# lucidrains/dreamer4

Hardware: AMD Instinct MI355X
Metric: imagined latent steps/sec (higher is better)
Workload: dtype f32; 1 GPU; cfg2 Moving-MNIST-latent shape: dim=512 depth=6 heads=8x64 latents=32x32 spatial=4 registers=8; generate(H+1=16 frames, num_steps=4, time cache) + learn_from_experience(ppo) + clip/AdamW both heads; global_batch=256, per_gpu_batch=256, horizon=15, num_steps=4, parallelism=dp1

## Files before the change

### dreamer4_amd/_lib.py

```python
from __future__ import annotations

import ctypes as C
import os

_HERE = os.path.dirname(os.path.abspath(__file__))
LIB_PATH = os.path.join(_HERE, 'libd4hip.so')

D4_MAX_ACTION_TYPES = 8

GEMM_RMS_ROWSCALE, GEMM_SILU, GEMM_SWIGLU, GEMM_TRANS_A, GEMM_TRANS_B, GEMM_ACCUMULATE = 1, 2, 4, 8, 16, 32


class Config(C.Structure):
    _fields_ = [
        ('dim', C.c_int32), ('dim_latent', C.c_int32), ('num_latent_tokens', C.c_int32), ('depth', C.c_int32),
        ('time_block_every', C.c_int32), ('attn_heads', C.c_int32), ('attn_dim_head', C.c_int32),
        ('attn_softclamp_value', C.c_float),
        ('num_spatial_tokens', C.c_int32), ('num_register_tokens', C.c_int32), ('max_steps', C.c_int32),
        ('num_tasks', C.c_int32), ('num_discrete_action_types', C.c_int32),
        ('num_discrete_actions', C.c_int32 * D4_MAX_ACTION_TYPES), ('num_continuous_actions', C.c_int32),
        ('multi_token_pred_len', C.c_int32),
        ('policy_head_mlp_depth', C.c_int32), ('value_head_mlp_depth', C.c_int32),
        ('terminal_mlp_depth', C.c_int32), ('predict_terminals', C.c_int32),
        ('reward_num_bins', C.c_int32), ('value_num_bins', C.c_int32), ('reward_encoder_type', C.c_int32), ('matmul_bf16', C.c_int32), ('head_mlp_recipe', C.c_int32), ('continuous_beta_param', C.c_int32),
# ... 168 lines not shown
    'd4_gemm_split': (_I, [_P, _I, _P, _L, _I, _P, _I, _P, _P, _I, _I, _I, _I, _I, _F, _I, _P]),
    'd4_split_f16x2': (_I, [_P, _P, _I, _I, _I, _L, _P, _P]),
    'd4_row_scale_exp': (_I, [_P, _L, _I, _I, _P, _P]),
    'd4_gemm_split2': (_I, [_P, _I, _P, _L, _I, _P, _P, _I, _P, _P, _I, _I, _I, _I, _I, _F, _I, _P, _P]),
    'd4_rmsnorm': (_I, [_P, _I, _P, _P, _I, _I, _I, _F, _P]),
    'd4_small_attn': (_I, [_P, _L, _L] * 4 + [_P] + [_P, _L, _L] * 3 + [_P] + [_I] * 4 + [_F] + [_I] * 6 + [_P]),
    'd4_small_attn_wide': (_I, [_P, _L, _L] * 4 + [_P] + [_P, _L, _L] * 3 + [_P] + [_I] * 4 + [_F] + [_I] * 6 + [_P]),
    'd4_small_attn_wide_bf16': (_I, [_P, _L, _L] * 4 + [_P] + [_P, _L, _L] * 3 + [_P] + [_I] * 4 + [_F] + [_I] * 6 + [_P]),
    'd4_pool_mix': (_I, [_P, _I, _P, _I, _P, _P, _I, _P, _I, _P, _P, _I, _I, _I, _F, _P, _P, _P, _P, _P]),
    'd4_pool_mix_deep': (_I, [_P, _I, _P, _I, _P, _P, _I, _P, _I, _P, _P, _I, _I, _I, _F, _P, _P, _P, _P, _P]),
    'd4_time_attn_decode': (_I, [_P, _I, _P, _I, _P, _P, _P, _P, _I, _P] + [_I] * 8 + [_P, _F, _I, _I, _P]),
    'd4_gemm_family_configs': (_I, [_I]),
    'd4_gemm_run': (_I, [C.POINTER(GemmDesc), _I, _I, _P]),
    'd4_gemm_run_rowmap': (_I, [C.POINTER(GemmDesc), _I, _I, _I, _I, _I, _I, _P]),
    'd4_gemm_run_pair': (_I, [C.POINTER(GemmDesc), C.POINTER(GemmDesc), _I, _I, _P]),
    'd4_gemm_fill_capacity': (_I, [C.POINTER(GemmDesc)]),
    'd4_gemm_run_fill': (_I, [C.POINTER(GemmDesc), C.POINTER(GemmDesc), _I, _P]),
    'd4_gemm_run_fill_rowmap': (_I, [C.POINTER(GemmDesc), C.POINTER(GemmDesc), _I, _I, _I, _I, _I, _P]),
    'd4_tile16_weights': (_I, [_P, _I, _P, _I, _I, _P]),
    'd4_frame_attn_out': (_I, [_P, _L, _L] * 4 + [_P] + [_P, _L, _L] * 2 + [_P] + [_I] * 3 + [_F] + [_I] * 3 + [_P, _I, _P, _I, _P, _I, _P, _I, _I, _I, _I, _P]),
    'd4_attn_out_cols': (_I, [_P, _L, _L] * 4 + [_P] + [_P, _L, _L] * 2 + [_P] + [_I] * 3 + [_F] + [_I] * 3 + [_P, _I, _I, _P, _I, _P, _I, _P, _I, _I, _I, _I, _P]),
    'd4_frame_pool': (_I, [_P, _I, _P, _I, _P, _P, _I, _P, _I, _P, _I, _I, _I, _F, _P, _P, _I, _I, _P, _I, _P, _I, _P, _I, _I, _I, _I, _P]),
    'd4_frame_pool_tail': (_I, [_P, _P, _P, _I, _I, _I, _I, _P, _I, _P, _I, _P, _I, _I, _I, _I, _P]),
    'd4_lqap_in': (_I, [_P, _I, _P, _I, _P, _P, _P, _P] + [_I] * 5 + [_F, _P]),
    'd4_lqap_out': (_I, [_P, _I, _P, _P, _P, _P, _I, _P, _I] + [_I] * 5 + [_P]),
    'd4_debug_last_form': (C.c_char_p, [C.c_char_p]),
    'd4_debug_forms': (_I, [C.c_char_p, _I, C.POINTER(C.c_char_p)]),
    'd4_train_attn_core_plane_floats': (C.c_size_t, [_I] * 3),
    'd4_train_xattn_core_plane_floats': (C.c_size_t, [_I] * 4),
    'd4_train_attn_core': (_I, [_P, _I] + [_P] * 7 + [_I] * 4 + [_F, _I, _I, _I, _L, _L, _I, _P, _I, _P, C.c_size_t, _P]),
# ... 90 lines not shown
```

### dreamer4_amd/csrc/abi_ops.hip

```cpp
#include "common.h"
#include "engine.h"
#include "prof.h"

extern "C" {

int d4_profile_bf16_enable(int stride) { d4::gemm_bf16_profile_enable(stride); return 0; }
int d4_profile_bf16_read(double* ms, double* flops, int64_t* count) { return d4::gemm_bf16_profile_read(ms, flops, count); }
int d4_profile_enable(int on) { return d4::gemm_profile_enable(on); }
int d4_profile_read(double* ms, double* flops, int64_t* count, int nclass) { return d4::gemm_profile_read(ms, flops, count, nclass); }
int d4_profile_classes(void) { return d4::gemm_profile_classes(); }
int d4_profile_glue_enable(int mask) { return d4::glue_profile_enable(mask); }
int d4_profile_glue_read(double* ms, double* bytes, int64_t* count, int nclass) { return d4::glue_profile_read(ms, bytes, count, nclass); }
int d4_profile_glue_classes(void) { return d4::GL_N; }
int d4_profile_glue_read_flops(double* flops, int nclass) { return d4::glue_profile_read_flops(flops, nclass); }
const char* d4_profile_glue_class_name(int c) { return d4::glue_class_name(c); }
int d4_frame_fused_set(int mode) { return d4::frame_fused_set(mode); }
const char* d4_profile_class_name(int c) { return d4::gemm_profile_class_name(c); }

int d4_gemm(const float* A, int lda, const float* W, int ldw, float* C, int ldc, const float* bias,
            const float* R, int ldr, int M, int N, int K, int flags, float rms_eps, void* stream) {
    d4::GemmArgs g{A, lda, W, ldw, C, ldc, bias, R, ldr, M, N, K, flags, rms_eps};
    return d4::gemm(g, static_cast<hipStream_t>(stream));
}

// ... 403 lines not shown
            D4_REQUIRE(al16(a) && al16(b) && d4::gemm_skinny_pair_applicable(a, b),
                       "d4_gemm_run_pair: call not supported (gemm_skinny_pair_applicable: two few-row products of equal K, no SiLU-GLU, batch or mirror weights)");
            return d4::gemm_skinny_pair(a, b, s);
        case D4_PAIR_BF16A:
            D4_REQUIRE(d4::gemm_bf16a_pair_applicable(a, b),
                       "d4_gemm_run_pair: call not supported (gemm_bf16a_pair_applicable: equal K, flags == RMS, no bias / R / C2 / batch, a 64 x 64 or 128 x 64 tile by the rule)");
            return d4::gemm_bf16a_pair_launch(a, b, s);
        case D4_PAIR_V2:
            D4_REQUIRE(al16(a) && al16(b) && !a.Wb && !b.Wb && a.K == b.K && d4::gemm2_pair_config_ok(config) && d4::gemm2_pair_applicable(a, b) &&
                       d4::gemm2_config_valid(config, a) && d4::gemm2_config_valid(config, b),
                       "d4_gemm_run_pair: call not supported (gemm2 pair configuration %d: gemm2_pair_config_ok / gemm2_pair_applicable)", config);
            return d4::gemm2_pair_launch(config, a, b, s);
    }
    D4_REQUIRE(false, "d4_gemm_run_pair: unknown target %d", target);
}

int d4_tile16_weights(const float* W, int ldw, float* Wt, int N, int K, void* stream) {
    D4_REQUIRE(W && Wt && N >= 16 && K >= 4 && ldw >= K && ((uintptr_t)W % 16) == 0 && ((uintptr_t)Wt % 16) == 0, "d4_tile16_weights: bad arguments");
    return d4::tile16_weights(W, ldw, Wt, N, K, static_cast<hipStream_t>(stream));
}
static d4::SmallAttnArgs frame_attn_args(const float* q, int64_t q_group_stride, int64_t q_item_stride, const float* k, int64_t k_group_stride, int64_t k_item_stride,
                                         const float* v, int64_t v_group_stride, int64_t v_item_stride, const float* gate, int64_t g_group_stride, int64_t g_item_stride,
                                         const float* k_gamma, const float* vres, int64_t r_group_stride, int64_t r_item_stride, const float* mix, int64_t m_group_stride,
                                         int64_t m_item_stride, uint16_t* out_b, int frames, int heads, int S, float softclamp, int mask_special, int belief, int dh) {
    d4::SmallAttnArgs sa{};
    sa.q = q; sa.q_group_stride = q_group_stride; sa.q_item_stride = q_item_stride;
    sa.k = k; sa.k_group_stride = k_group_stride; sa.k_item_stride = k_item_stride;
    sa.v = v; sa.v_group_stride = v_group_stride; sa.v_item_stride = v_item_stride;
    sa.gate = gate; sa.g_group_stride = g_group_stride; sa.g_item_stride = g_item_stride;
    sa.k_gamma = k_gamma;
// ... 81 lines not shown
```

### dreamer4_amd/csrc/engine.hip

```cpp
#include "common.h"
#include "engine.h"
#include "prof.h"
#include <math.h>
#include <stdarg.h>
#include <stdio.h>
#include <stdlib.h>
#include <string.h>
#include <memory>

using namespace d4;

namespace d4 {

static constexpr float RMS_EPS = 1.1920928955078125e-07f;

static int round_up(int v, int m) { return (v + m - 1) / m * m; }

int engine_layout(d4_engine* e, bool assign) {
    const d4_config& c = e->c;
    size_t off = 0;
    auto alloc_bytes = [&](size_t bytes) -> char* {
        off = (off + 255) / 256 * 256;
        char* p = assign ? e->ws + off : nullptr;
        off += bytes;
// ... 725 lines not shown
    int32_t offs[D4_MAX_ACTION_TYPES] = {0}, sizes[D4_MAX_ACTION_TYPES] = {0};
    int o = 0;
    for (int a = 0; a < e->na; ++a) { offs[a] = o; sizes[a] = c.num_discrete_actions[a]; o += sizes[a]; }
    D4_HIP(hipMemcpyAsync(e->action_offsets, offs, sizeof(offs), hipMemcpyHostToDevice, s));
    D4_HIP(hipMemcpyAsync(e->action_sizes, sizes, sizeof(sizes), hipMemcpyHostToDevice, s));
    D4_HIP(hipStreamSynchronize(s));
    e->prepared = true;
    return 0;
}

static GemmArgs ff_in_call(const d4_engine* e, const FfPrep& fp, const float* x, int ldx, int rows) {
    return GemmArgs{x, ldx, fp.w1, e->D, e->ffh, e->inner_pad, fp.b1, nullptr, 0, rows, 2 * e->inner_pad, e->D,
                    GEMM_RMS_ROWSCALE | GEMM_SWIGLU, RMS_EPS, 2.0 * rows * (2.0 * e->inner) * e->D};
}

static int ff_block(const EvalCtx& cx, d4_engine* e, const FfPrep& fp, const float* out_b, const float* x, int ldx, float* y, int ldy,
                    int rows, float* y_compact = nullptr, int S = 0, int has_agent = 1, const GemmArgs* fill = nullptr) {
    int rc;
    GemmArgs g1 = ff_in_call(e, fp, x, ldx, rows);
    if (fill) {
        trunk_call(cx.img, g1);
        if ((rc = gemm_x3sk_fill(g1, *fill, gemm_x3sk_fill_tiles(*fill), cx.s))) return rc;
    } else
    if ((rc = engine_gemm(cx, g1))) return rc;
    GemmArgs g2{e->ffh, e->inner_pad, fp.w2, e->inner_pad, y, ldy, out_b, x, ldx, rows, e->D, e->inner_pad, 0, RMS_EPS,
                2.0 * rows * (double)e->D * e->inner};
    if (y_compact) { g2.C2 = y_compact; g2.ldc2 = e->D; g2.c2_S = S; g2.c2_lo = cx.keep_lo; g2.c2_hi = cx.keep_hi; g2.c2_last = has_agent; }
    return engine_gemm(cx, g2);
}

int g_pool_wide_keys = 1;
int g_rollout_clean_agent_row = 1;
int g_rollout_batched_heads = 1;
int g_lqap_in_fused = 1;
int g_lqap_out_fused = 1;
int g_last_layer_compact_q = 1;
int g_layer0_const_rows = 1;
int g_pool_const_keys = 1;
int g_ff_fill_pool_keys = 1;
unsigned g_launch_count = 0;
static GemmArgs pool_key_call(d4_engine* e, int p, const float* hiddens, int L, int M, int rule_M, float* keys0) {
    const int D = e->D, hp = e->hp;
    GemmArgs gk{hiddens, D, e->pkv_w[p], D, e->pool_kv, hp, nullptr, nullptr, 0, L * M, hp, D, GEMM_RMS_ROWSCALE, RMS_EPS};
    gk.rule_M = L * rule_M;
    if (keys0) { gk.A = hiddens + (size_t)M * D; gk.C = keys0 + (size_t)M * hp; gk.M = (L - 1) * M; gk.rule_M = L * M; }
    return gk;
}

static int pool_block(const EvalCtx& cx, d4_engine* e, int p, const float* x, float* y, int L, int M, const float* hiddens = nullptr,
                      float* y_compact = nullptr, int S = 0, int has_agent = 1, int rule_M = 0, float* keys0 = nullptr, int keys_done = 0) {
    if (!hiddens) hiddens = e->slabs;
    const d4_config& c = e->c;
    const int D = e->D, hp = e->hp;
    const AttnW& a = e->pools[p];
// ... 266 lines not shown
            GemmArgs g1 = ff_in_call(e, e->ffp[l], h1, D, M);
            trunk_call(cx.img, g1);
            const int cap = gemm_rule_takes_x3sk(g1) ? gemm_x3sk_fill_capacity(g1) : 0;
            const GemmArgs gk = pool_key_call(e, l, e->slabs, L, M, 0, keys0(l));
            const int ready = (gk.M - M) / 128;
            const int per_block = (e->hp + 63) / 64;
            const int blocks = cap / per_block < ready ? cap / per_block : ready;
            if (blocks > 0 && takes(v2, L * M, e->hp, D, GEMM_RMS_ROWSCALE, e->pkv_w[l]) &&
                takes(v2, gk.M - 128 * blocks, e->hp, D, GEMM_RMS_ROWSCALE, e->pkv_w[l], L * M)) {
                keys_done = 128 * blocks;
                kfill = gk;
                kfill.M = keys_done; kfill.rule_M = 0;
                D4_REQUIRE(gemm_x3sk_fill_applicable(kfill), "ff_fill_pool_keys: the key problem of pool %d is no fill problem", l);
            }
        }
        if ((rc = ff_block(cx, e, e->ffp[l], e->layer_ff[l].out_b, h1, D, h2, D, M, cslab(2 * l + 2), S, has_agent, keys_done ? &kfill : nullptr))) return rc;
        if (l != c.depth - 1) {
            float* xc = compact_tail_at(l + 1) ? e->xpool_c : nullptr;
            if ((rc = pool_block(cx, e, l, h2, e->xpool, 2 * l + 3, M, nullptr, xc, S, has_agent, 0, keys0(l), keys_done))) return rc;
            x_in = e->xpool;
        }
    }

    float* xfc = e->xfc;
    const float* last = slab(2 * c.depth);
    if ((rc = copy_rows(cslab(2 * c.depth), D, xfc, D, Mc, D, s))) return rc;
    if (e->encoder) {
        const int P = e->P;
        const float* spec = cslab(2 * c.depth);
        if ((rc = gemm_simple(cx, spec, D, e->cq_w, D, e->cq, e->ldcq, Mc, hd + h, D, GEMM_RMS_ROWSCALE, nullptr, nullptr, 0))) return rc;
        if ((rc = gemm_simple(cx, last, D, e->ckv_w, D, e->ckv, 2 * hd, M, 2 * hd, D, GEMM_RMS_ROWSCALE, nullptr, nullptr, 0))) return rc;
        SmallAttnArgs sa{};
        sa.dh = c.attn_dim_head;
        sa.q = e->cq; sa.q_group_stride = (int64_t)n * e->ldcq; sa.q_item_stride = e->ldcq;
// ... 404 lines not shown
    D4_REQUIRE(!io->sample_actions || e->nc == 0 || (io->actions_cont && io->beta_noise && io->log_probs_cont && io->cont_params), "sample_actions needs the continuous action outputs and beta_noise");
    D4_REQUIRE(!io->sample_actions || io->values, "sample_actions needs the values output");
    D4_REQUIRE(!io->sample_terminals || (c.predict_terminals && io->bern_u), "sample_terminals needs predict_terminals and bern_u");
    D4_REQUIRE(io->use_time_cache || io->noise_context || T - P <= 1, "noise_context is required without the time cache");
    const int F = T - P;
    const int step_size = c.max_steps / K;
    int sl, rc;
    if ((rc = step_log2_of(step_size, &sl))) return rc;
    if ((rc = check_step_log2(e, sl))) return rc;
    const int n_el = c.num_latent_tokens * c.dim_latent;
    const int D = e->D, S = e->S, A = e->A, na = e->na, nc = e->nc;
    if (!io->use_time_cache) e->cache_frames = 0;
    const bool lean = d4::g_rollout_clean_agent_row != 0;
    const int lean_keep = (lean && d4::engine_clean_agent_only(e)) ? 1 : c.num_spatial_tokens + 1;
    const int variant = (lean ? 1 : 0) | (d4::g_lqap_in_fused ? 2 : 0) | (d4::g_lqap_out_fused ? 4 : 0) | (d4::g_last_layer_compact_q ? 8 : 0) |
                        (d4::g_layer0_const_rows ? 16 : 0) | (d4::g_pool_const_keys ? 32 : 0) | (d4::g_ff_fill_pool_keys ? 64 : 0);
    const float* hist = nullptr;
    if (d4::g_rollout_batched_heads && F >= 1 && F <= e->head_rows) {
        if (io->agent_embed) hist = io->agent_embed;
        else if (F == 1) hist = e->agent_c;
        else if ((size_t)B * F <= e->hist_rows) hist = e->agent_hist;
    }
    const bool heads_after = hist != nullptr;

    for (int f = 0; f < F; ++f) {
        const int cur = P + f;
        int Tq, t0;
        bool commit;
        if (io->use_time_cache && (e->cache_frames > 0 || cur == 0)) { Tq = 1; t0 = e->cache_frames; commit = true; }
        else if (io->use_time_cache) { Tq = cur + 1; t0 = 0; commit = true; }
        else { Tq = cur + 1; t0 = 0; commit = false; }
// ... 122 lines not shown
}


int d4_debug_switch(const char* name, int value) {
    int* sw = nullptr;
    if (name && !strcmp(name, "launch_count")) {
        const int old = (int)(d4::g_launch_count & 0x7fffffffu);
        d4::g_launch_count = (unsigned)value;
        return old;
    }
    if (name && !strcmp(name, "ff_fill_launches")) {
        const int old = (int)(d4::g_fill_launches & 0x7fffffffu);
        d4::g_fill_launches = (unsigned)value;
        return old;
    }
    if (name && !strcmp(name, "time_attn_fused_append")) sw = &d4::g_time_attn_fused_append;
    else if (name && !strcmp(name, "rollout_clean_agent_row")) sw = &d4::g_rollout_clean_agent_row;
    else if (name && !strcmp(name, "rollout_batched_heads")) sw = &d4::g_rollout_batched_heads;
    else if (name && !strcmp(name, "attn_out_cols")) sw = &d4::g_attn_out_cols;
    else if (name && !strcmp(name, "lqap_in_fused")) sw = &d4::g_lqap_in_fused;
    else if (name && !strcmp(name, "lqap_out_fused")) sw = &d4::g_lqap_out_fused;
    else if (name && !strcmp(name, "last_layer_compact_q")) sw = &d4::g_last_layer_compact_q;
    else if (name && !strcmp(name, "layer0_const_rows")) sw = &d4::g_layer0_const_rows;
    else if (name && !strcmp(name, "pool_const_keys")) sw = &d4::g_pool_const_keys;
    else if (name && !strcmp(name, "ff_fill_pool_keys")) sw = &d4::g_ff_fill_pool_keys;
    else if (name && !strcmp(name, "pool_wide_keys")) sw = &d4::g_pool_wide_keys;
    else if (name && !strcmp(name, "pool_mix_deep")) sw = &d4::g_pool_mix_deep;
    else if (name && !strcmp(name, "time_attn_tiled")) sw = &d4::g_time_attn_tiled;
    else if (name && !strcmp(name, "space_attn_tiled")) sw = &d4::g_space_attn_tiled;
    else if (name && !strcmp(name, "cross_attn_tiled")) sw = &d4::g_cross_attn_tiled;
    else if (name && !strcmp(name, "small_attn_wide")) sw = &d4::g_small_attn_wide;
    if (!sw) return -1;
    const int old = *sw;
    *sw = value;
    return old;
}
int d4_gemm_force_config(int id) {
    d4::gemm_bf16a_force_config(-1);
    d4::gemm_bf16_force_config(-1);
    const int n_main = d4::gemm_force_config(-1);
// ... 33 lines not shown
```

### dreamer4_amd/csrc/gemm.hip

```cpp
#include "common.h"
#include <string.h>
#include <hip/hip_ext.h>
#include "kernels.h"
#include <mutex>
#include <math.h>
#include <stdio.h>
#include <stdlib.h>
#include <map>
#include <tuple>
#include <type_traits>
#include <vector>

namespace d4 {


template <int BM, int BN, int WGM, int WGN, int BK, int KS, bool TA, bool TB, bool KTAIL>
__global__ __launch_bounds__(WGM * WGN * 64 * KS) void gemm_kernel(GemmArgs p) {
    constexpr int LDS_LD = BK + 4;
    constexpr int RF4 = BK / 4;
    constexpr int NT = WGM * WGN * 64 * KS;
    constexpr int TM = BM / WGM / 32;
    constexpr int TN = BN / WGN / 32;
    static_assert(TM >= 1 && TN >= 1, "tile");
    constexpr int A_F4 = BM * BK / 4 / NT;
// ... 797 lines not shown
    D4_TUNE_STRICT_CHECK(p, nb);
    int best = 0;
    if (int rc = autotune_v4(p, stream, &best)) return rc;
    g_tuned4[key] = best;
    tune_cache_append(key, 400 + best);
    return launch_v4(best, p, stream);
}

bool gemm_h2_takes(const GemmArgs& p) {
    if (!p.Wb || p.wplane <= 0 || !p.wscale || !gemm_h2_applicable(p) || gemm_skinny_applicable(p)) return false;
    if (g_forced_cfg >= 0 && g_forced_cfg < 400) return false;
    if (g_forced_cfg >= 400) return true;
    return p.M >= 256 && p.K >= 128 && p.N >= 64 && (double)p.M * p.N * p.K * (p.batch > 0 ? p.batch : 1) >= 1.2e9;
}

int gemm_pair(const GemmArgs& a_in, const GemmArgs& b_in, hipStream_t stream) {
    std::lock_guard<std::recursive_mutex> lock(gemm_mutex());
    GemmArgs a = a_in, b = b_in;
    if (int rc = gemm_rowmap_refused(a, "gemm_pair")) return rc;
    if (int rc = gemm_rowmap_refused(b, "gemm_pair")) return rc;
    const bool fp32_rule = (!a.Wb || (a.wplane > 0 && a.N < 2048)) && (!b.Wb || (b.wplane > 0 && b.N < 2048)) &&
                           !gemm_h2_takes(a) && !gemm_h2_takes(b);
    if (fp32_rule && g_forced_cfg < 0 && a.M > 0 && b.M > 0 && a.K == b.K && use_v2(a) && use_v2(b) && !gemm_skinny_applicable(a) &&
        !gemm_skinny_applicable(b) && gemm2_pair_applicable(a, b)) {
        a.Wb = nullptr; a.wplane = 0; a.wscale = nullptr; b.Wb = nullptr; b.wplane = 0; b.wscale = nullptr;
        const GemmArgs& big = (double)a.M * a.N >= (double)b.M * b.N ? a : b;
        tune_cache_load();
        auto it = g_tuned2.find(TuneKey{big.M, big.N, big.K, big.flags, big.batch});
        const int c = it != g_tuned2.end() ? it->second : heuristic_v2(big);
        if (gemm2_pair_config_ok(c) && gemm2_config_valid(c, a) && gemm2_config_valid(c, b)) {
            const int cls = N_TILE_CFG + c;
            const bool timed = ((g_prof_mask >> cls) & 1) && (g_prof_tick++ % g_prof_stride) == 0;
            if (!timed) return gemm2_pair_launch(c, a, b, stream);
            ProfRec rec{};
            rec.a = prof_event(); rec.b = prof_event(); rec.cls = cls;
// ... 97 lines not shown
```

### dreamer4_amd/csrc/gemm2.hip

```cpp
#include "common.h"
#include <hip/hip_ext.h>
#include "kernels.h"
#include "gemm2_body.h"
#include <stdlib.h>
#include <type_traits>

namespace d4 {

template <int WGM, int WGN, int TM, int TN, int NS, int BK, bool RMS>
__global__ __launch_bounds__(WGM* WGN * 64) void gemm2_kernel(GemmArgs p) {
    gemm2_body<WGM, WGN, TM, TN, NS, BK, RMS>(p, blockIdx.x, blockIdx.y);
}

template <int WGM, int WGN, int TM, int TN, int NS, int BK, bool RMS>
__global__ __launch_bounds__(WGM* WGN * 64) void gemm2_rowmap_kernel(GemmArgs p) {
    gemm2_body<WGM, WGN, TM, TN, NS, BK, RMS, true>(p, blockIdx.x, blockIdx.y);
}

template <int WGM, int WGN, int TM, int TN, int NS, int BK, bool RMS>
__global__ __launch_bounds__(WGM* WGN * 64) void gemm2_pair_kernel(GemmArgs a, GemmArgs b, int nblk_a) {
    const int bid = blockIdx.x;
    if (bid < nblk_a) gemm2_body<WGM, WGN, TM, TN, NS, BK, RMS>(a, bid, 0);
    else gemm2_body<WGM, WGN, TM, TN, NS, BK, RMS>(b, bid - nblk_a, 0);
}

constexpr int KS_GROUPS = 4, KS_NS = 3, KS_BM = 32, KS_BN = 64, KS_BK = 32;
constexpr int KS_STAGE_F = (KS_BM + KS_BN) * KS_BK;
constexpr int KS_RING_F = KS_NS * KS_STAGE_F;
constexpr int KS_LDP = KS_BN + 4;

__global__ __launch_bounds__(1024) void gemm2_ksplit_kernel(GemmArgs p) {
    constexpr int BK = KS_BK, CH = 8, RPP = 8, BM = KS_BM, BN = KS_BN, NS = KS_NS, LPW = 3, NSLOT = (BM + BN) / RPP;
    extern __shared__ __attribute__((aligned(16))) float smem[];
    const int tid = threadIdx.x, lane = tid & 63;
    const int wave = __builtin_amdgcn_readfirstlane(tid >> 6);
    const int grp = wave >> 2, w = wave & 3, wm = w >> 1, wn = w & 1;
    int bid = blockIdx.x;
    const int nbn = (p.N + BN - 1) / BN, nbm = (p.M + BM - 1) / BM;
// ... 206 lines not shown
int gemm2_pair_launch(int c, const GemmArgs& a, const GemmArgs& b, hipStream_t stream, hipEvent_t ea, hipEvent_t eb) {
    if (int rc = gemm_rowmap_refused(a, "gemm2 pair")) return rc;
    if (int rc = gemm_rowmap_refused(b, "gemm2 pair")) return rc;
    D4_REQUIRE(gemm2_pair_applicable(a, b) && gemm2_config_valid(c, a) && gemm2_config_valid(c, b), "gemm2 pair: configuration %d is not valid for these calls", c);
    switch (c) {
        case V2_64x64: return launch2_pair<2, 2, 2, 2, 3, 32>(a, b, stream, ea, eb);
        case V2_128x64_8: return launch2_pair<4, 2, 2, 2, 3, 32>(a, b, stream, ea, eb);
        case V2_128x64_k16: return launch2_pair<4, 2, 2, 2, 4, 16>(a, b, stream, ea, eb);
        case V2_32x64: return launch2_pair<2, 2, 1, 2, 3, 32>(a, b, stream, ea, eb);
        case V2_32x32: return launch2_pair<2, 2, 1, 1, 3, 32>(a, b, stream, ea, eb);
        case V2_64x32: return launch2_pair<4, 1, 1, 2, 3, 32>(a, b, stream, ea, eb);
    }
    return 2;
}

int gemm2_launch(int c, const GemmArgs& p, hipStream_t stream, hipEvent_t ea, hipEvent_t eb) {
    D4_REQUIRE(gemm2_config_valid(c, p), "gemm2: configuration %d is not valid for this call", c);
    switch (c) {
        case V2_64x64: return launch2<2, 2, 2, 2, 3, 32>(p, stream, ea, eb);
        case V2_64x64_s: return launch2<4, 1, 1, 4, 3, 32>(p, stream, ea, eb);
        case V2_128x64_8: return launch2<4, 2, 2, 2, 3, 32>(p, stream, ea, eb);
        case V2_128x64_s: return launch2<4, 1, 2, 4, 3, 32>(p, stream, ea, eb);
        case V2_128x64_k16: return launch2<4, 2, 2, 2, 4, 16>(p, stream, ea, eb);
        case V2_128x128_k16: return launch2<4, 2, 2, 4, 3, 16>(p, stream, ea, eb);
        case V2_32x64: return launch2<2, 2, 1, 2, 3, 32>(p, stream, ea, eb);
        case V2_32x64_s: return launch2<2, 1, 1, 4, 3, 32>(p, stream, ea, eb);
        case V2_32x32: return launch2<2, 2, 1, 1, 3, 32>(p, stream, ea, eb);
        case V2_64x32: return launch2<4, 1, 1, 2, 3, 32>(p, stream, ea, eb);
    }
    return 2;
// ... 4 lines not shown
```

### dreamer4_amd/csrc/kernels.h

```cpp
#pragma once
#include <hip/hip_runtime.h>
#include <stdint.h>

namespace d4 {

enum : int {
    GEMM_RMS_ROWSCALE = 1,
    GEMM_SILU = 2,
    GEMM_SWIGLU = 4,
    GEMM_TRANS_A = 8,
    GEMM_TRANS_B = 16,
    GEMM_ACCUMULATE = 32,
};

struct GemmArgs {
    const float* A; int lda;
    const float* W; int ldw;
    float* C; int ldc;
    const float* bias;
    const float* R; int ldr;
    int M, N, K;
    int flags;
    float rms_eps;
    double algo_flops = 0;
// ... 67 lines not shown
int gemm_x3sk_fill_launch(const GemmArgs& main, const GemmArgs& fill, int fill_tiles, hipStream_t stream, hipEvent_t ea = nullptr, hipEvent_t eb = nullptr);
extern unsigned g_fill_launches;
int gemm_x3sk_fill(const GemmArgs& main, const GemmArgs& fill, int fill_tiles, hipStream_t stream);
bool gemm2_applicable(const GemmArgs& p);
bool gemm2_config_valid(int c, const GemmArgs& p);
int gemm2_configs();
const char* gemm2_config_name(int c);
void gemm2_config_tile(int c, int* bm, int* bn);
int gemm2_launch(int c, const GemmArgs& p, hipStream_t stream, hipEvent_t ea = nullptr, hipEvent_t eb = nullptr);
bool gemm2_ksplit_applicable(const GemmArgs& p);
bool gemm2_ksplit_rule(const GemmArgs& p);
int gemm2_ksplit_launch(const GemmArgs& p, hipStream_t stream, hipEvent_t ea = nullptr, hipEvent_t eb = nullptr);
bool gemm2_pair_config_ok(int c);
bool gemm2_pair_applicable(const GemmArgs& a, const GemmArgs& b);
int gemm2_pair_launch(int c, const GemmArgs& a, const GemmArgs& b, hipStream_t stream, hipEvent_t ea = nullptr, hipEvent_t eb = nullptr);
int gemm_pair(const GemmArgs& a, const GemmArgs& b, hipStream_t stream);
bool gemm_skinny_applicable(const GemmArgs& p);
int gemm_skinny(const GemmArgs& p, hipStream_t stream);
bool gemm_skinny_pair_applicable(const GemmArgs& a, const GemmArgs& b);
int gemm_skinny_pair(const GemmArgs& a, const GemmArgs& b, hipStream_t stream);
int gemm_profile_enable(int on);
bool gemm_profile_active();
int gemm_profile_read(double* ms, double* flops, int64_t* count, int nclass);
int gemm_profile_classes();
extern int g_time_attn_fused_append;
extern int g_pool_wide_keys;
extern int g_attn_out_cols;
extern int g_time_attn_tiled;
extern int g_space_attn_tiled;
extern int g_cross_attn_tiled;
extern int g_small_attn_wide;
// ... 211 lines not shown
```

### include/d4hip.h

```cpp
#ifndef D4HIP_H
#define D4HIP_H

#include <stddef.h>
#include <stdint.h>

#ifdef __cplusplus
extern "C" {
#endif

#define D4_MAX_ACTION_TYPES 8
#define D4_MODE_DYNAMICS 0
#define D4_MODE_DECODER 1
#define D4_MODE_ENCODER 2
#define D4_MLP_PRE_RMS 0
#define D4_MLP_POST_LAYER 1
#define D4_BETA_SOFTPLUS_P1 0
#define D4_BETA_EXP_P1 1

typedef struct d4_config {
    int32_t dim, dim_latent, num_latent_tokens, depth, time_block_every;
    int32_t attn_heads, attn_dim_head;
    float attn_softclamp_value;
    int32_t num_spatial_tokens, num_register_tokens, max_steps, num_tasks;
    int32_t num_discrete_action_types;
// ... 309 lines not shown
#define D4_GEMM_H2 5
#define D4_GEMM_SKINNY 6
#define D4_GEMM_BF16 7
#define D4_GEMM_BF16A 8
#define D4_GEMM_FAMILIES 9
int d4_gemm_family_configs(int family);
int d4_gemm_run(const d4_gemm_desc* d, int family, int config, void* stream);
int d4_gemm_run_rowmap(const d4_gemm_desc* d, int family, int config, int rm_Sc, int rm_S, int rm_lo, int rm_nr, void* stream);
int d4_gemm_fill_capacity(const d4_gemm_desc* main_call);
int d4_gemm_run_fill(const d4_gemm_desc* main_call, const d4_gemm_desc* fill, int fill_tiles, void* stream);
int d4_gemm_run_fill_rowmap(const d4_gemm_desc* main_call, const d4_gemm_desc* fill, int fill_tiles, int rm_Sc, int rm_S, int rm_lo, int rm_nr, void* stream);
#define D4_PAIR_SKINNY 0
#define D4_PAIR_BF16A 1
#define D4_PAIR_V2 2
int d4_gemm_run_pair(const d4_gemm_desc* a, const d4_gemm_desc* b, int target, int config, void* stream);
int d4_tile16_weights(const float* W, int ldw, float* Wt, int N, int K, void* stream);
int d4_frame_attn_out(const float* q, int64_t q_group_stride, int64_t q_item_stride, const float* k, int64_t k_group_stride, int64_t k_item_stride,
                      const float* v, int64_t v_group_stride, int64_t v_item_stride, const float* gate, int64_t g_group_stride, int64_t g_item_stride,
                      const float* k_gamma, const float* vres, int64_t r_group_stride, int64_t r_item_stride, const float* mix, int64_t m_group_stride,
                      int64_t m_item_stride, uint16_t* out_b, int frames, int heads, int S, float softclamp, int mask_special, int belief, int dh,
                      const float* wo_t, int D, const float* resid, int ldr, float* out, int ldo, float* c2, int ldc2, int c2_lo, int c2_hi, int c2_last,
                      void* stream);
int d4_attn_out_cols(const float* q, int64_t q_group_stride, int64_t q_item_stride, const float* k, int64_t k_group_stride, int64_t k_item_stride,
                     const float* v, int64_t v_group_stride, int64_t v_item_stride, const float* gate, int64_t g_group_stride, int64_t g_item_stride,
                     const float* k_gamma, const float* vres, int64_t r_group_stride, int64_t r_item_stride, const float* mix, int64_t m_group_stride,
                     int64_t m_item_stride, uint16_t* out_b, int frames, int heads, int S, float softclamp, int mask_special, int belief, int dh,
                     const float* W, int ldw, int D, const float* resid, int ldr, float* out, int ldo, float* c2, int ldc2, int c2_lo, int c2_hi, int c2_last,
                     void* stream);
int d4_frame_pool(const float* q, int ldq, const float* x, int ldx, const float* gate_w, const float* k, int ldk, const float* hid, int D,
                  const float* k_gamma, int M, int L, int heads, float eps, const float* wv_t, const float* wo_t, int frames, int S, const float* resid,
// ... 135 lines not shown
```

Before: 23620 imagined steps/s.

## Pair FF output GEMM with old pool-key GEMM in one mixed-RMS launch

Adds a paired GEMM kernel where one half runs without the RMS row scale and the other with it. In the dynamics forward pass it uses this kernel to compute the pool-key projection of older rows together with the feed-forward output GEMM of each non-final layer. The aim is fewer launches and better occupancy from co-scheduling a skinny GEMM with a larger independent one. In exchange it adds another kernel variant, a switch, and extra eligibility checks on the host.

Result: no change. 23810 imagined steps/s (median of 6 runs) (+0.8%).

```diff
diff --git a/dreamer4_amd/_lib.py b/dreamer4_amd/_lib.py
--- a/dreamer4_amd/_lib.py
+++ b/dreamer4_amd/_lib.py
@@ -206,6 +206,8 @@
     'd4_gemm_run': (_I, [C.POINTER(GemmDesc), _I, _I, _P]),
     'd4_gemm_run_rowmap': (_I, [C.POINTER(GemmDesc), _I, _I, _I, _I, _I, _I, _P]),
     'd4_gemm_run_pair': (_I, [C.POINTER(GemmDesc), C.POINTER(GemmDesc), _I, _I, _P]),
+    'd4_gemm_run_pair_mixed': (_I, [C.POINTER(GemmDesc), C.POINTER(GemmDesc), _I, _P]),
+    'd4_gemm_run_pair_mixed_rowmap': (_I, [C.POINTER(GemmDesc), C.POINTER(GemmDesc), _I, _I, _I, _I, _I, _P]),
     'd4_gemm_fill_capacity': (_I, [C.POINTER(GemmDesc)]),
     'd4_gemm_run_fill': (_I, [C.POINTER(GemmDesc), C.POINTER(GemmDesc), _I, _P]),
     'd4_gemm_run_fill_rowmap': (_I, [C.POINTER(GemmDesc), C.POINTER(GemmDesc), _I, _I, _I, _I, _I, _P]),
diff --git a/dreamer4_amd/csrc/abi_ops.hip b/dreamer4_amd/csrc/abi_ops.hip
--- a/dreamer4_amd/csrc/abi_ops.hip
+++ b/dreamer4_amd/csrc/abi_ops.hip
@@ -441,6 +441,24 @@
     }
     D4_REQUIRE(false, "d4_gemm_run_pair: unknown target %d", target);
 }
+static int gemm_run_pair_mixed_args(const d4::GemmArgs& a, const d4::GemmArgs& b, int config, void* stream) {
+    auto al16 = [](const d4::GemmArgs& g) { return ((uintptr_t)g.A % 16) == 0 && ((uintptr_t)g.W % 16) == 0 && (g.lda % 4) == 0 && (g.ldw % 4) == 0; };
+    D4_REQUIRE(al16(a) && al16(b) && !a.Wb && !b.Wb, "d4_gemm_run_pair_mixed: call not supported (operands must be 16-byte aligned f32 matrices, no mirror weights)");
+    return d4::gemm2_pair_mixed_launch(config, a, b, static_cast<hipStream_t>(stream));
+}
+int d4_gemm_run_pair_mixed(const d4_gemm_desc* da, const d4_gemm_desc* db, int config, void* stream) {
+    if (int rc = gemm_desc_check("d4_gemm_run_pair_mixed", da)) return rc;
+    if (int rc = gemm_desc_check("d4_gemm_run_pair_mixed", db)) return rc;
+    return gemm_run_pair_mixed_args(gemm_args_of(*da), gemm_args_of(*db), config, stream);
+}
+int d4_gemm_run_pair_mixed_rowmap(const d4_gemm_desc* da, const d4_gemm_desc* db, int config, int rm_Sc, int rm_S, int rm_lo, int rm_nr, void* stream) {
+    if (int rc = gemm_desc_check("d4_gemm_run_pair_mixed_rowmap", da)) return rc;
+    if (int rc = gemm_desc_check("d4_gemm_run_pair_mixed_rowmap", db)) return rc;
+    D4_REQUIRE(rm_Sc >= 1 && rm_nr >= 0 && rm_lo >= 0 && rm_lo <= rm_Sc && rm_S == rm_Sc + rm_nr && rm_S <= 65535, "d4_gemm_run_pair_mixed_rowmap: bad row map (Sc=%d S=%d lo=%d nr=%d)", rm_Sc, rm_S, rm_lo, rm_nr);
+    d4::GemmArgs b = gemm_args_of(*db);
+    b.rm_Sc = (uint16_t)rm_Sc; b.rm_lo = (uint16_t)rm_lo; b.rm_nr = (uint16_t)rm_nr;
+    return gemm_run_pair_mixed_args(gemm_args_of(*da), b, config, stream);
+}
 
 int d4_tile16_weights(const float* W, int ldw, float* Wt, int N, int K, void* stream) {
     D4_REQUIRE(W && Wt && N >= 16 && K >= 4 && ldw >= K && ((uintptr_t)W % 16) == 0 && ((uintptr_t)Wt % 16) == 0, "d4_tile16_weights: bad arguments");
diff --git a/dreamer4_amd/csrc/engine.hip b/dreamer4_amd/csrc/engine.hip
--- a/dreamer4_amd/csrc/engine.hip
+++ b/dreamer4_amd/csrc/engine.hip
@@ -763,8 +763,16 @@
                     GEMM_RMS_ROWSCALE | GEMM_SWIGLU, RMS_EPS, 2.0 * rows * (2.0 * e->inner) * e->D};
 }
 
+static GemmArgs ff_out_call(const EvalCtx& cx, const d4_engine* e, const FfPrep& fp, const float* out_b, const float* x, int ldx, float* y, int ldy, int rows,
+                            float* y_compact, int S, int has_agent) {
+    GemmArgs g2{e->ffh, e->inner_pad, fp.w2, e->inner_pad, y, ldy, out_b, x, ldx, rows, e->D, e->inner_pad, 0, RMS_EPS,
+                2.0 * rows * (double)e->D * e->inner};
+    if (y_compact) { g2.C2 = y_compact; g2.ldc2 = e->D; g2.c2_S = S; g2.c2_lo = cx.keep_lo; g2.c2_hi = cx.keep_hi; g2.c2_last = has_agent; }
+    return g2;
+}
+
 static int ff_block(const EvalCtx& cx, d4_engine* e, const FfPrep& fp, const float* out_b, const float* x, int ldx, float* y, int ldy,
-                    int rows, float* y_compact = nullptr, int S = 0, int has_agent = 1, const GemmArgs* fill = nullptr) {
+                    int rows, float* y_compact = nullptr, int S = 0, int has_agent = 1, const GemmArgs* fill = nullptr, const GemmArgs* old_keys = nullptr) {
     int rc;
     GemmArgs g1 = ff_in_call(e, fp, x, ldx, rows);
     if (fill) {
@@ -772,9 +780,12 @@
         if ((rc = gemm_x3sk_fill(g1, *fill, gemm_x3sk_fill_tiles(*fill), cx.s))) return rc;
     } else
     if ((rc = engine_gemm(cx, g1))) return rc;
-    GemmArgs g2{e->ffh, e->inner_pad, fp.w2, e->inner_pad, y, ldy, out_b, x, ldx, rows, e->D, e->inner_pad, 0, RMS_EPS,
-                2.0 * rows * (double)e->D * e->inner};
-    if (y_compact) { g2.C2 = y_compact; g2.ldc2 = e->D; g2.c2_S = S; g2.c2_lo = cx.keep_lo; g2.c2_hi = cx.keep_hi; g2.c2_last = has_agent; }
+    GemmArgs g2 = ff_out_call(cx, e, fp, out_b, x, ldx, y, ldy, rows, y_compact, S, has_agent);
+    if (old_keys) {
+        GemmArgs gk = *old_keys;
+        trunk_call(cx.img, g2); trunk_call(cx.img, gk);
+        return gemm_pair(g2, gk, cx.s);
+    }
     return engine_gemm(cx, g2);
 }
 
@@ -787,6 +798,7 @@
 int g_layer0_const_rows = 1;
 int g_pool_const_keys = 1;
 int g_ff_fill_pool_keys = 1;
+int g_ff_out_pool_keys = 1;
 unsigned g_launch_count = 0;
 static GemmArgs pool_key_call(d4_engine* e, int p, const float* hiddens, int L, int M, int rule_M, float* keys0) {
     const int D = e->D, hp = e->hp;
@@ -1083,10 +1095,25 @@
                 D4_REQUIRE(gemm_x3sk_fill_applicable(kfill), "ff_fill_pool_keys: the key problem of pool %d is no fill problem", l);
             }
         }
-        if ((rc = ff_block(cx, e, e->ffp[l], e->layer_ff[l].out_b, h1, D, h2, D, M, cslab(2 * l + 2), S, has_agent, keys_done ? &kfill : nullptr))) return rc;
+        GemmArgs kold{};
+        int keys_old = 0;
+        if (g_ff_out_pool_keys && dynamics && e->split && l < c.depth - 1 && e->pool_mix_path() && !e->kall_b) {
+            const int L = 2 * l + 3;
+            const GemmArgs gk = pool_key_call(e, l, e->slabs, L, M, 0, keys0(l));
+            const int old = gk.M - M - keys_done;
+            if (old >= 128 && takes(v2, L * M, e->hp, D, GEMM_RMS_ROWSCALE, e->pkv_w[l]) && takes(v2, M, e->hp, D, GEMM_RMS_ROWSCALE, e->pkv_w[l], L * M)) {
+                GemmArgs gb = gk;
+                gb.A += (size_t)keys_done * D; gb.C += (size_t)keys_done * e->hp; gb.M = old; gb.rule_M = L * M;
+                GemmArgs ta = ff_out_call(cx, e, e->ffp[l], e->layer_ff[l].out_b, h1, D, h2, D, M, cslab(2 * l + 2), S, has_agent), tb = gb;
+                trunk_call(cx.img, ta); trunk_call(cx.img, tb);
+                if (gemm_pair_takes_mixed(ta, tb)) { kold = gb; keys_old = old; }
+            }
+        }
+        if ((rc = ff_block(cx, e, e->ffp[l], e->layer_ff[l].out_b, h1, D, h2, D, M, cslab(2 * l + 2), S, has_agent, keys_done ? &kfill : nullptr,
+                           keys_old ? &kold : nullptr))) return rc;
         if (l != c.depth - 1) {
             float* xc = compact_tail_at(l + 1) ? e->xpool_c : nullptr;
-            if ((rc = pool_block(cx, e, l, h2, e->xpool, 2 * l + 3, M, nullptr, xc, S, has_agent, 0, keys0(l), keys_done))) return rc;
+            if ((rc = pool_block(cx, e, l, h2, e->xpool, 2 * l + 3, M, nullptr, xc, S, has_agent, 0, keys0(l), keys_done + keys_old))) return rc;
             x_in = e->xpool;
         }
     }
@@ -1521,7 +1548,8 @@
     const bool lean = d4::g_rollout_clean_agent_row != 0;
     const int lean_keep = (lean && d4::engine_clean_agent_only(e)) ? 1 : c.num_spatial_tokens + 1;
     const int variant = (lean ? 1 : 0) | (d4::g_lqap_in_fused ? 2 : 0) | (d4::g_lqap_out_fused ? 4 : 0) | (d4::g_last_layer_compact_q ? 8 : 0) |
-                        (d4::g_layer0_const_rows ? 16 : 0) | (d4::g_pool_const_keys ? 32 : 0) | (d4::g_ff_fill_pool_keys ? 64 : 0);
+                        (d4::g_layer0_const_rows ? 16 : 0) | (d4::g_pool_const_keys ? 32 : 0) | (d4::g_ff_fill_pool_keys ? 64 : 0) |
+                        (d4::g_ff_out_pool_keys ? 128 : 0);
     const float* hist = nullptr;
     if (d4::g_rollout_batched_heads && F >= 1 && F <= e->head_rows) {
         if (io->agent_embed) hist = io->agent_embed;
@@ -1674,6 +1702,11 @@
         d4::g_fill_launches = (unsigned)value;
         return old;
     }
+    if (name && !strcmp(name, "ff_out_keys_launches")) {
+        const int old = (int)(d4::g_pair_mixed_launches & 0x7fffffffu);
+        d4::g_pair_mixed_launches = (unsigned)value;
+        return old;
+    }
     if (name && !strcmp(name, "time_attn_fused_append")) sw = &d4::g_time_attn_fused_append;
     else if (name && !strcmp(name, "rollout_clean_agent_row")) sw = &d4::g_rollout_clean_agent_row;
     else if (name && !strcmp(name, "rollout_batched_heads")) sw = &d4::g_rollout_batched_heads;
@@ -1684,6 +1717,7 @@
     else if (name && !strcmp(name, "layer0_const_rows")) sw = &d4::g_layer0_const_rows;
     else if (name && !strcmp(name, "pool_const_keys")) sw = &d4::g_pool_const_keys;
     else if (name && !strcmp(name, "ff_fill_pool_keys")) sw = &d4::g_ff_fill_pool_keys;
+    else if (name && !strcmp(name, "ff_out_pool_keys")) sw = &d4::g_ff_out_pool_keys;
     else if (name && !strcmp(name, "pool_wide_keys")) sw = &d4::g_pool_wide_keys;
     else if (name && !strcmp(name, "pool_mix_deep")) sw = &d4::g_pool_mix_deep;
     else if (name && !strcmp(name, "time_attn_tiled")) sw = &d4::g_time_attn_tiled;
diff --git a/dreamer4_amd/csrc/gemm.hip b/dreamer4_amd/csrc/gemm.hip
--- a/dreamer4_amd/csrc/gemm.hip
+++ b/dreamer4_amd/csrc/gemm.hip
@@ -835,11 +835,37 @@
     return p.M >= 256 && p.K >= 128 && p.N >= 64 && (double)p.M * p.N * p.K * (p.batch > 0 ? p.batch : 1) >= 1.2e9;
 }
 
+static int pair_mixed_config(const GemmArgs& a, const GemmArgs& b) {
+    if (a.M < 1 || b.M < 1 || a.rm_Sc > 0 || b.rm_Sc > 0 || !gemm2_pair_mixed_applicable(a, b) || !gemm_rule_takes_v2(a) || !gemm_rule_takes_v2(b)) return -1;
+    tune_cache_load();
+    auto it = g_tuned2.find(TuneKey{a.M, a.N, a.K, a.flags, a.batch});
+    const int c = it != g_tuned2.end() && gemm2_pair_mixed_config_ok(it->second) ? it->second : heuristic_v2(a);
+    return gemm2_pair_mixed_config_ok(c) && gemm2_config_valid(c, a) && gemm2_config_valid(c, b) ? c : -1;
+}
+bool gemm_pair_takes_mixed(const GemmArgs& a, const GemmArgs& b) {
+    std::lock_guard<std::recursive_mutex> lock(gemm_mutex());
+    return pair_mixed_config(a, b) >= 0;
+}
+
 int gemm_pair(const GemmArgs& a_in, const GemmArgs& b_in, hipStream_t stream) {
     std::lock_guard<std::recursive_mutex> lock(gemm_mutex());
     GemmArgs a = a_in, b = b_in;
     if (int rc = gemm_rowmap_refused(a, "gemm_pair")) return rc;
     if (int rc = gemm_rowmap_refused(b, "gemm_pair")) return rc;
+    if (const int c = pair_mixed_config(a, b); c >= 0) {
+        a.Wb = nullptr; a.wplane = 0; a.wscale = nullptr; a.aexp = nullptr; b.Wb = nullptr; b.wplane = 0; b.wscale = nullptr; b.aexp = nullptr;
+        const int cls = N_TILE_CFG + c;
+        const bool timed = ((g_prof_mask >> cls) & 1) && (g_prof_tick++ % g_prof_stride) == 0;
+        if (!timed) return gemm2_pair_mixed_launch(c, a, b, stream);
+        ProfRec rec{};
+        rec.a = prof_event(); rec.b = prof_event(); rec.cls = cls;
+        rec.M = a.M + b.M; rec.N = a.N; rec.K = a.K; rec.flags = a.flags; rec.batch = 2;
+        gemm2_config_tile(c, &rec.bm, &rec.bn);
+        rec.flops = (a.algo_flops > 0 ? a.algo_flops : 2.0 * a.M * a.N * a.K) + (b.algo_flops > 0 ? b.algo_flops : 2.0 * b.M * b.N * b.K);
+        if (int rc = gemm2_pair_mixed_launch(c, a, b, stream, rec.a, rec.b)) return rc;
+        g_prof.push_back(rec);
+        return 0;
+    }
     const bool fp32_rule = (!a.Wb || (a.wplane > 0 && a.N < 2048)) && (!b.Wb || (b.wplane > 0 && b.N < 2048)) &&
                            !gemm_h2_takes(a) && !gemm_h2_takes(b);
     if (fp32_rule && g_forced_cfg < 0 && a.M > 0 && b.M > 0 && a.K == b.K && use_v2(a) && use_v2(b) && !gemm_skinny_applicable(a) &&
diff --git a/dreamer4_amd/csrc/gemm2.hip b/dreamer4_amd/csrc/gemm2.hip
--- a/dreamer4_amd/csrc/gemm2.hip
+++ b/dreamer4_amd/csrc/gemm2.hip
@@ -22,6 +22,13 @@
     const int bid = blockIdx.x;
     if (bid < nblk_a) gemm2_body<WGM, WGN, TM, TN, NS, BK, RMS>(a, bid, 0);
     else gemm2_body<WGM, WGN, TM, TN, NS, BK, RMS>(b, bid - nblk_a, 0);
+}
+
+template <int WGM, int WGN, int TM, int TN, int NS, int BK, bool RMS_A, bool RMS_B>
+__global__ __launch_bounds__(WGM* WGN * 64) void gemm2_pair_mixed_kernel(GemmArgs a, GemmArgs b, int nblk_a) {
+    const int bid = blockIdx.x;
+    if (bid < nblk_a) gemm2_body<WGM, WGN, TM, TN, NS, BK, RMS_A>(a, bid, 0);
+    else gemm2_body<WGM, WGN, TM, TN, NS, BK, RMS_B>(b, bid - nblk_a, 0);
 }
 
 constexpr int KS_GROUPS = 4, KS_NS = 3, KS_BM = 32, KS_BN = 64, KS_BK = 32;
@@ -258,6 +265,49 @@
     return 2;
 }
 
+unsigned g_pair_mixed_launches = 0;
+
+template <int WGM, int WGN, int TM, int TN, int NS, int BK>
+static int launch2_pair_mixed(const GemmArgs& a, const GemmArgs& b, hipStream_t stream, hipEvent_t ea, hipEvent_t eb) {
+    constexpr int BM = WGM * TM * 16, BN = WGN * TN * 16;
+    const size_t lds = (size_t)(NS * (BM + BN) * BK + BM) * sizeof(float);
+    auto k = gemm2_pair_mixed_kernel<WGM, WGN, TM, TN, NS, BK, false, true>;
+    static DeviceOnce attr_set;
+    if (attr_set.need()) {
+        D4_HIP(hipFuncSetAttribute(reinterpret_cast<const void*>(k), hipFuncAttributeMaxDynamicSharedMemorySize, (int)lds));
+        attr_set.done();
+    }
+    const int64_t na = (int64_t)cdiv(a.M, BM) * cdiv(a.N, BN), nb = (int64_t)cdiv(b.M, BM) * cdiv(b.N, BN);
+    D4_REQUIRE(na + nb <= 0x7FFFFFFF, "gemm2 mixed pair: %lld blocks exceed the grid", (long long)(na + nb));
+    const dim3 grid((unsigned)(na + nb)), block(WGM * WGN * 64);
+    if (ea) hipExtLaunchKernelGGL(k, grid, block, (uint32_t)lds, stream, ea, eb, 0, a, b, (int)na);
+    else hipLaunchKernelGGL(k, grid, block, lds, stream, a, b, (int)na);
+    D4_LAUNCH_CHECK();
+    ++g_pair_mixed_launches;
+    return 0;
+}
+
+bool gemm2_pair_mixed_config_ok(int c) { return c == V2_64x64 || c == V2_32x64 || c == V2_128x64_8; }
+
+bool gemm2_pair_mixed_applicable(const GemmArgs& a, const GemmArgs& b) {
+    return gemm2_applicable(a) && gemm2_applicable(b) && a.batch <= 1 && b.batch <= 1 && !(a.flags & GEMM_RMS_ROWSCALE) && (b.flags & GEMM_RMS_ROWSCALE) &&
+           !(a.flags & GEMM_SWIGLU) && !(b.flags & GEMM_SWIGLU) && a.rm_Sc == 0 && b.rm_Sc == 0;
+}
+
+int gemm2_pair_mixed_launch(int c, const GemmArgs& a, const GemmArgs& b, hipStream_t stream, hipEvent_t ea, hipEvent_t eb) {
+    if (int rc = gemm_rowmap_refused(a, "gemm2 mixed pair")) return rc;
+    if (int rc = gemm_rowmap_refused(b, "gemm2 mixed pair")) return rc;
+    D4_REQUIRE(gemm2_pair_mixed_config_ok(c) && gemm2_pair_mixed_applicable(a, b) && gemm2_config_valid(c, a) && gemm2_config_valid(c, b),
+               "gemm2 mixed pair: call not supported (configuration %d; a: M=%d N=%d K=%d flags=%d batch=%d, b: M=%d N=%d K=%d flags=%d batch=%d — a without and "
+               "b with the row scale, no SiLU-GLU, batch or row map)", c, a.M, a.N, a.K, a.flags, a.batch, b.M, b.N, b.K, b.flags, b.batch);
+    switch (c) {
+        case V2_64x64: return launch2_pair_mixed<2, 2, 2, 2, 3, 32>(a, b, stream, ea, eb);
+        case V2_128x64_8: return launch2_pair_mixed<4, 2, 2, 2, 3, 32>(a, b, stream, ea, eb);
+        case V2_32x64: return launch2_pair_mixed<2, 2, 1, 2, 3, 32>(a, b, stream, ea, eb);
+    }
+    return 2;
+}
+
 int gemm2_launch(int c, const GemmArgs& p, hipStream_t stream, hipEvent_t ea, hipEvent_t eb) {
     D4_REQUIRE(gemm2_config_valid(c, p), "gemm2: configuration %d is not valid for this call", c);
     switch (c) {
diff --git a/dreamer4_amd/csrc/kernels.h b/dreamer4_amd/csrc/kernels.h
--- a/dreamer4_amd/csrc/kernels.h
+++ b/dreamer4_amd/csrc/kernels.h
@@ -105,7 +105,12 @@
 bool gemm2_pair_config_ok(int c);
 bool gemm2_pair_applicable(const GemmArgs& a, const GemmArgs& b);
 int gemm2_pair_launch(int c, const GemmArgs& a, const GemmArgs& b, hipStream_t stream, hipEvent_t ea = nullptr, hipEvent_t eb = nullptr);
+bool gemm2_pair_mixed_config_ok(int c);
+bool gemm2_pair_mixed_applicable(const GemmArgs& a, const GemmArgs& b);
+int gemm2_pair_mixed_launch(int c, const GemmArgs& a, const GemmArgs& b, hipStream_t stream, hipEvent_t ea = nullptr, hipEvent_t eb = nullptr);
+extern unsigned g_pair_mixed_launches;
 int gemm_pair(const GemmArgs& a, const GemmArgs& b, hipStream_t stream);
+bool gemm_pair_takes_mixed(const GemmArgs& a, const GemmArgs& b);
 bool gemm_skinny_applicable(const GemmArgs& p);
 int gemm_skinny(const GemmArgs& p, hipStream_t stream);
 bool gemm_skinny_pair_applicable(const GemmArgs& a, const GemmArgs& b);
diff --git a/include/d4hip.h b/include/d4hip.h
--- a/include/d4hip.h
+++ b/include/d4hip.h
@@ -347,6 +347,8 @@
 #define D4_PAIR_BF16A 1
 #define D4_PAIR_V2 2
 int d4_gemm_run_pair(const d4_gemm_desc* a, const d4_gemm_desc* b, int target, int config, void* stream);
+int d4_gemm_run_pair_mixed(const d4_gemm_desc* a, const d4_gemm_desc* b, int config, void* stream);
+int d4_gemm_run_pair_mixed_rowmap(const d4_gemm_desc* a, const d4_gemm_desc* b, int config, int rm_Sc, int rm_S, int rm_lo, int rm_nr, void* stream);
 int d4_tile16_weights(const float* W, int ldw, float* Wt, int N, int K, void* stream);
 int d4_frame_attn_out(const float* q, int64_t q_group_stride, int64_t q_item_stride, const float* k, int64_t k_group_stride, int64_t k_item_stride,
                       const float* v, int64_t v_group_stride, int64_t v_item_stride, const float* gate, int64_t g_group_stride, int64_t g_item_stride,
```
